# mit-acl/dpgo

Measured on AMD Instinct MI355X. Metric: rbcd_iterations_per_sec, higher is better.
Workload: dtype f64; 1 GPU; synthetic 3-D grid 50x50x40 (100000 poses, 293500 edges), init = perturbed truth; agents=1, agents_per_gpu=1, r=5, d=3, schedule=single agent, poses_per_agent=100000, nnzb_per_agent=687000

## Files before the change

dpgo_amd/csrc/host.h:

```cpp
#pragma once
#include "kernels.h"
#include "handoff.h"
#include "options.h"
#include "taskpool.h"
#include "aggregation.h"

#include <algorithm>
#include <atomic>
#include <chrono>
#include <condition_variable>
#include <functional>
#include <memory>
#include <pthread.h>
#include <sched.h>
#include <mutex>
#include <thread>
#include <type_traits>
#include <cmath>
#include <cstdio>
#include <cstdlib>
#include <cstring>
#include <string>
#include <utility>
#include <vector>
// ... 312 lines not shown
  }
  bool beyond_cache() const {
    return sizeof(double) * ((size_t)Q.nnzb * b * b + 8 * (size_t)n * T) + sizeof(int32_t) * (size_t)Q.nnzb + loop_extra_bytes >
           ((size_t)256 << 20);
  }
  bool persist = false;
  int persist_share = 1;
  int persist_wgs = 0, persist_split = 0, persist_mt = 0;
  int persist_reserved = 0;
  bool persist_failed_once = false;
  bool stream_nt = false;
  bool persist_add = false;
  bool persist_stream_ordered = false;
  struct Pending {
    bool active = false;
    bool launched = false;
    SolvePlan plan;
    BorrowedIterate x;
    dpgo_ropt_result result{};
  } pending;
  DevBuf<PersistCtrl> pctrl;
  bool pctrl_dirty = true;
  DevBuf<unsigned long long> pgran;
  unsigned gran_cleared_at = 0;
  PinBuf<PersistCtrl> hctrl;
  DevBuf<double> partial_mem;
  Partials pE, pA, pB, pH;
  DevBuf<DevState> state_mem;
  StateSlots<DevState> state;
  PinBuf<DevState> hstate;
  PinBuf<unsigned long long> hflag;
  unsigned gen = 0;
  bool saw_rtr_stop = false;
  struct GncEdges {
    int em = 0;
    DevBuf<int32_t> e_p1, e_p2, c_ptr, c_edge;
    DevBuf<double> e_R, e_t, e_kappa, e_tau, e_w, e_rsq, q_base;
    DevBuf<uint8_t> e_fixed, c_kind, e_role;
    DevBuf<int32_t> e_slot;
    DevBuf<int32_t> g_ptr, g_edge;
    DevBuf<uint8_t> g_kind;
    DevBuf<double> c_base;
    int n_shared_edges = 0;
    DevBuf<RobustPartial> r_partial;
    DevBuf<RobustStatsDev> r_stats;
    EdgeDev dev() const {
      return EdgeDev{e_p1, e_p2, e_R, e_t, e_kappa, e_tau, e_fixed, e_role, e_slot, e_w, e_rsq, em};
    }
  } gnc;
  size_t vec_bytes() const { return (size_t)n * T * sizeof(double); }
  int grid() const { return std::min(pose_tiles(n, b), cap_u); }
  int cap_u = kMaxGrid, cap_h = kMaxGrid;
  int cap_u_ml = kMaxGrid;
  int grid_u(bool ml_mode) const { return std::min(pose_tiles(n, b), ml_mode ? cap_u_ml : cap_u); }
  int split = 1;
  int grid_s() const { return std::min(pose_tiles(n, b, split), tcg_sym ? cap_hs : cap_h); }
  int cap_restrict = kMaxGrid, cap_post = kMaxGrid;
  int grid_restrict() const { return std::min(pose_tiles(n, b, split), cap_restrict); }
  int grid_post() const { return std::min(pose_tiles(n, b, split), cap_post); }
  int cap_outer_sym = kMaxGrid;
  int grid_outer_sym() const { return std::min(pose_tiles(n, b), cap_outer_sym); }
  int cap_spmm_sym = kMaxGrid;
  int grid_spmm_sym() const { return std::min(pose_tiles(n, b), cap_spmm_sym); }
  int grid_spmm() const { return std::min(pose_tiles(n, b, split), kMaxGrid); }
  int grid_flat() const {
    size_t total = (size_t)n * T;
// ... 112 lines not shown
```

dpgo_amd/csrc/kernels/common.h:

```cpp
#pragma once


constexpr int kBlock = 256;
constexpr int kWaves = kBlock / 64;
constexpr int kMaxGrid = 1024;
constexpr int kPartialCap = 1024;
constexpr int kNP = 4;

enum : int { TCG_NEGCURV = 0, TCG_EXCREGION = 1, TCG_LCON = 2, TCG_SCON = 3, TCG_MAXITER = 4 };

struct DevState {
  double f1, ngf, Delta, Delta_max, tol;
  double f2, rho, fInit, gnInit;
  double xqx, xg;
  int outer_iter, rtr_stop, accepted_last, n_accept;
  int accept_tiny, pad0;
  double z_r, d_Pd, e_Pd, e_Pe, norm_r0, alpha, theta, kappa;
  double d_Hd;
  int tcg_j, tcg_done, tcg_status, max_inner;
  int n_hess, min_inner;
};

__device__ __forceinline__ void publish_progress(unsigned long long* hflag, unsigned gen, const DevState& st) {
  if (hflag) {
    const unsigned long long w = ((unsigned long long)gen << 32) |
                                 ((unsigned long long)((unsigned)st.tcg_j & 0xFFFFFFu) << 8) |
                                 (st.rtr_stop ? 2ull : 0ull) | (st.tcg_done ? 1ull : 0ull);
    __hip_atomic_store(hflag, w, __ATOMIC_RELAXED, __HIP_MEMORY_SCOPE_SYSTEM);
  }
}

__device__ __forceinline__ unsigned state_gen(DevState& st, unsigned gen) {
  if (gen) st.pad0 = (int)gen;
  return (unsigned)st.pad0;
}

#define DPGO_STATE_FIELDS(X)                                                                              \
  X(f1) X(ngf) X(Delta) X(Delta_max) X(tol) X(f2) X(rho) X(fInit) X(gnInit) X(xqx) X(xg) X(outer_iter)      \
  X(rtr_stop) X(accepted_last) X(n_accept) X(accept_tiny) X(pad0) X(z_r) X(d_Pd) X(e_Pd) X(e_Pe) X(norm_r0) \
  X(alpha) X(theta) X(kappa) X(d_Hd) X(tcg_j) X(tcg_done) X(tcg_status) X(max_inner) X(n_hess) X(min_inner)
__device__ __forceinline__ void load_state(DevState& st, const DevState* __restrict__ p) {
#define X(f) st.f = p->f;
  DPGO_STATE_FIELDS(X)
#undef X
}
__device__ __forceinline__ void store_state(DevState* __restrict__ p, const DevState& st) {
#define X(f) p->f = st.f;
  DPGO_STATE_FIELDS(X)
#undef X
}

template <int D, int R, int SPLIT = 1>
struct Geo {
  static constexpr int B = D + 1;
  static constexpr int T = B * R;
  static constexpr int BB = B * B;
  static constexpr int LPP = B * SPLIT;
  static constexpr int G = 64 / LPP;
  static constexpr int P = G * kWaves;
};
// ... 692 lines not shown
```

dpgo_amd/csrc/kernels/multilevel.h:

```cpp
#pragma once


struct AggMap {
  const int32_t* lab;
  int k;
  __device__ __forceinline__ int of(int i) const { return lab ? lab[i] : i / k; }
};

template <int D, int R>
__global__ __launch_bounds__(kBlock) void k_ml_presmooth(const double* __restrict__ V, const double* __restrict__ dinv,
                                                         double omega, double* __restrict__ OUT,
                                                         const DevState* __restrict__ gate, int n) {
  using GEO = Geo<D, R>;
  if (gate && (gate->tcg_done || gate->rtr_stop)) return;
  __shared__ double sm[kWaves][GEO::G][GEO::T];
  const LaneId L = lane_id<D>();
  const int ntiles = (n + GEO::P - 1) / GEO::P;
  const TileIter ti_ = tile_iter(ntiles);
  for (int tile = ti_.first; tile < ti_.last; tile += ti_.step) {
    const int i = tile * GEO::P + L.wave * GEO::G + L.g;
    const bool ok = (L.g < GEO::G) && (i < n);
    const size_t off = (size_t)i * GEO::T + L.c * R;
    double* vs = ok ? &sm[L.wave][L.g][0] : nullptr;
    double v[R], z[R];
// ... 21 lines not shown
};
template <int D, int R, int SPLIT>
struct RestrictWaves {
  static constexpr int kMin = (SPLIT == 1 && D == 3 && R <= 5) ? DPGO_RESTRICT_WAVES : 1;
};
template <int D, int R, int SPLIT, class MAT = BsrDev, class PT = double, class XT = double>
__global__ __launch_bounds__(kBlock) __attribute__((amdgpu_waves_per_eu(RestrictWaves<D, R, SPLIT>::kMin, 8))) void k_ml_restrict(MAT A, const XT* __restrict__ x1,
                                                        const double* __restrict__ r, const PT* __restrict__ Pb,
                                                        double shift, int k, double* __restrict__ rc,
                                                        float* __restrict__ rc32,
                                                        const double* __restrict__ dinv_next, double omega,
                                                        double* __restrict__ x1c, const DevState* gate,
                                                        int n, XT* __restrict__ res_out = nullptr,
                                                        double* __restrict__ tbuf = nullptr,
                                                        const int32_t* __restrict__ tpos = nullptr,
                                                        TcgStopCheck stop = TcgStopCheck()) {
  using GEO = Geo<D, R, SPLIT>;
  DPGO_TL_TILES_DECL;
  if (gate && (gate->tcg_done || gate->rtr_stop)) return;
  DPGO_STAMP_ENTRY_IN(g_tl_restrict);
  __shared__ double res_s[kWaves][GEO::G][GEO::T];
  __shared__ double t_s[GEO::P][GEO::T];
  const LaneId L = lane_id<D, SPLIT>();
  const int ntiles = (n + GEO::P - 1) / GEO::P;
  const TileIter ti_ = tile_iter(ntiles);
  if (stop.state && blockIdx.x == gridDim.x - 1) {
    double rr_sum[1];
    load_partials<1>(stop.pin, stop.nb, rr_sum, &t_s[0][0]);
    if (threadIdx.x == 0) {
      const DevState* st = stop.state;
      const double norm_r = sqrt(rr_sum[0]), nr0 = st->norm_r0, theta = st->theta, kappa = st->kappa;
      const double pw = (theta == 1.0) ? nr0 : pow(nr0, theta);
      const int j = st->tcg_j;
      if (j >= st->min_inner && norm_r <= nr0 * (pw < kappa ? pw : kappa)) {
        stop.state->tcg_status = (kappa < pw) ? TCG_LCON : TCG_SCON;
        stop.state->tcg_done = 1;
        if (stop.hflag) {
          const unsigned g_ = stop.gen ? stop.gen : (unsigned)st->pad0;
          const unsigned long long w = ((unsigned long long)g_ << 32) |
                                       ((unsigned long long)((unsigned)j & 0xFFFFFFu) << 8) | 1ull;
          __hip_atomic_store(stop.hflag, w, __ATOMIC_RELAXED, __HIP_MEMORY_SCOPE_SYSTEM);
        }
      }
    }
    __syncthreads();
  }
  DPGO_STAMP_AT_IN(g_tl_restrict, 1);
  for (int tk = ti_.first; tk < ti_.last; tk += ti_.step) {
    DPGO_STAMP_TILE_IN(g_tl_restrict, 0);
    const int tile = tile_of(A, tk);
    const int lp = L.wave * GEO::G + L.g;
    const int i = tile * GEO::P + lp;
    const bool okp = (L.g < GEO::G) && (i < n);
    const bool ok = okp && (L.s == 0);
    const size_t off = (size_t)i * GEO::T + L.c * R;
    double h[R];
    q_gather<D, R, SPLIT>(A, x1, i, L.s, L.c, okp, h);
    DPGO_TL_USE(h[0]);
    DPGO_STAMP_TILE_IN(g_tl_restrict, 1);
    if (ok) {
      XT xr[R];
      double rr[R];
#pragma unroll
      for (int a = 0; a < R; ++a) xr[a] = x1[off + a];
      load_col<R>(r + off, rr);
#pragma unroll
      for (int a = 0; a < R; ++a) h[a] = rr[a] - h[a] - shift * (double)xr[a];
      store_col<R>(&res_s[L.wave][L.g][L.c * R], h);
      if (res_out) store_col_t<R>(res_out + off, h);
    }
    wave_sync();
    DPGO_STAMP_TILE_IN(g_tl_restrict, 2);
    if (L.s == 0 && L.g < GEO::G) {
      double t[R];
#pragma unroll
// ... 793 lines not shown
```

dpgo_amd/csrc/solve.hip:

```cpp
#include "host.h"

namespace dpgo_host {

int launch_tcg_update(dpgo_problem_s* p, const double* dinv, int first, double* z_out,
                      double ml_omega) {
  const bool ml_mode = ml_omega > 0.0;
  const int g = p->grid_u(ml_mode);
  if (!first) CHK(sums_ready(p->pA));
  double* pb = nullptr;
  CHK(sums_out(p->pB, g, &pb));
  double* zt = z_out ? z_out : p->z;
  float* z32 = (ml_omega > 0.0 && !p->ml.empty() && z_out == p->ml[0].x1 && p->ml_vec32_active()) ? p->ml[0].x1f : nullptr;
  CHK(dispatch_dr(p->d, p->r, [&](auto Dc, auto Rc) {
    constexpr int D = decltype(Dc)::value, R = decltype(Rc)::value;
    const bool def = p->dirs_on;
    auto go = [&](auto kernel, auto... z32_arg) {
      return launch(kernel, g, 0, p->stream, p->x1, p->g1, dinv, def ? nullptr : p->delta.get(), p->Hd,
                    def ? nullptr : p->eta.get(), p->rr, zt, p->pA.in(), p->pA.count(), pb, p->state.in(),
                    p->state.out(), first, p->n, p->hflag, p->gen, ml_omega, def ? p->dirs_coef.get() : nullptr,
                    z32_arg...);
    };
    if constexpr (Span<D, R, 1>::kOk) {
      if (def) return go(ml_mode ? k_tcg_update_span<D, R, 1, 1> : k_tcg_update_span<D, R, 0, 1>, z32);
      return go(ml_mode ? k_tcg_update_span<D, R, 1> : k_tcg_update_span<D, R, 0>, z32);
// ... 257 lines not shown
  HIPC(hipGetLastError());
  *used = true;
  return DPGO_OK;
}

void persist_report(dpgo_problem_s* p) {
  if (!options().persist_verbose) return;
  const double it = std::max<double>(1.0, (double)p->hctrl->ticks[4]);
  std::fprintf(stderr,
               "dpgo_hip: persistent tCG: %u workgroups (%d lane groups per pose, %d tiles each)%s, %u iterations; per "
               "iteration (us): Hessian phase %.2f, all-reduce %.2f, update phase %.2f, all-reduce %.2f; per solve (us): "
               "set-up + initial statistics %.1f, first updates %.1f, retraction / trial point / rho test %.1f\n",
               p->hctrl->members, p->persist_split, p->persist_mt, p->hctrl->error ? " TIMED OUT" : "", p->hctrl->iters,
               0.01 * (double)p->hctrl->ticks[0] / it, 0.01 * (double)p->hctrl->ticks[1] / it,
               0.01 * (double)p->hctrl->ticks[2] / it, 0.01 * (double)p->hctrl->ticks[3] / it,
               0.01 * (double)p->hctrl->ticks[5], 0.01 * (double)p->hctrl->ticks[6], 0.01 * (double)p->hctrl->ticks[7]);
}

int rtr_outer_iteration(dpgo_problem_s* p, const dpgo_ropt_params* prm, const double* dinv, Counters& cnt,
                        bool poll_at_end) {
  p->gen += 1;
  const bool add = prm->precond == DPGO_PRECOND_ADDITIVE;
  const bool ml = prm->precond == DPGO_PRECOND_MULTILEVEL || add;
  if (add) cnt.vcycle_for_additive = true;
  auto update = [&](int first) -> int {
    if (ml) {
      CHK(launch_tcg_update(p, dinv, first, p->ml[0].x1, p->ml_omega));
      const bool early_stop = options().ml_early_stop != 0;
      return launch_ml_tail(p, p->x1, p->rr, p->z, &p->pB, p->state.in(), early_stop && !first);
    }
    return launch_tcg_update(p, dinv, first);
  };
  CHK(update(1));
  const int max_inner = prm->RTR_tCG_iterations;
  auto step = [&](int j) -> int {
    CHK(launch_tcg_hess(p, j == 0 ? 1 : 0));
    return update(0);
  };
  if (max_inner <= 0) CHK(launch_tcg_hess(p, 1));
  bool done = false;
  if (prm->tcg_poll_interval > 0) {
    const int poll = prm->tcg_poll_interval;
    int j = 0;
    while (j < max_inner) {
      const int chunk = (max_inner - j) < poll ? (max_inner - j) : poll;
      for (int c = 0; c < chunk; ++c) CHK(step(j + c));
      j += chunk;
      CHK(poll_state(p));
      if (p->hstate->tcg_done || p->hstate->rtr_stop) {
        done = true;
        break;
      }
    }
  } else {
    int kAhead = ml ? 2 : 4;
    if (options().tcg_ahead > 0) kAhead = std::max(2, options().tcg_ahead);
    int enq = 0, last_j = -1;
    auto t_progress = std::chrono::steady_clock::now();
    while (true) {
      const unsigned long long w = __atomic_load_n(p->hflag.get(), __ATOMIC_ACQUIRE);
      int dev_j = 0;
      if ((unsigned)(w >> 32) == p->gen) {
        dev_j = (int)((w >> 8) & 0xFFFFFFu);
        if (w & 3ull) {
          done = true;
          if (w & 2ull) p->saw_rtr_stop = true;
          break;
        }
      }
      if (enq >= max_inner) break;
      if (dev_j != last_j) {
        last_j = dev_j;
        t_progress = std::chrono::steady_clock::now();
      }
      if (enq < dev_j + kAhead) {
        CHK(step(enq));
        enq += 1;
      } else {
        __builtin_ia32_pause();
        if (std::chrono::duration<double>(std::chrono::steady_clock::now() - t_progress).count() > 60.0) {
          HIPC(hipStreamSynchronize(p->stream));
          return fail(DPGO_ERR_HIP, "tCG progress word did not advance for 60 s");
        }
      }
    }
  }
  if (!done) CHK(launch_tcg_hess(p, 0));
  if (p->saw_rtr_stop) return DPGO_OK;
  const bool rho_exact = options().rho_exact != 0;
  CHK(launch_retract(p, p->x1, p->eta, 1.0, p->x2, p->state.in(), rho_exact ? nullptr : p->rr.get(),
                     rho_exact ? nullptr : p->g1.get(), p->dirs_on));
  CHK(launch_grad(p, p->x2, p->g2, p->S2, nullptr, p->state.in(), p->tcg_sym && outer_sym_enabled()));
  cnt.spmm += 1;
  if (rho_exact) {
    CHK(launch_hess(p, p->x1, p->S1, p->eta, p->g1, p->Hd, p->state.in(), 0, p->tcg_sym && outer_sym_enabled()));
    cnt.spmm += 1;
  }
  CHK(launch_rtr_update(p));
  if (poll_at_end) CHK(poll_state(p));
  return DPGO_OK;
}

constexpr int kAutoUnitsJacobi = 10, kAutoUnitsAdditive = 13, kAutoSetupUnits = 2800, kAutoMinProducts = 6;
constexpr int kAutoUnitsAdditive2 = 22;
int auto_units_jacobi(dpgo_problem_s* p) {
  const int share = std::max(1, p->persist_share);
  if (share == 1 || !p->persist) return kAutoUnitsJacobi;
  const int cap = persist_capacity(p->device), limit = cap - cap / 5;
// ... 111 lines not shown
                     (prm->precond == DPGO_PRECOND_ADDITIVE || prm->precond == DPGO_PRECOND_BLOCK_JACOBI ||
                      prm->precond == DPGO_PRECOND_NONE);
  return DPGO_OK;
}

int one_launch_enqueue(dpgo_problem_s* p, const SolvePlan& plan, bool* used) {
  return launch_rtr_persistent(p, &plan.prm, plan.dinv, used, plan.prm.precond == DPGO_PRECOND_ADDITIVE);
}

int one_launch_collect(dpgo_problem_s* p, const SolvePlan& plan, dpgo_ropt_result* res, bool* ok) {
  *ok = false;
  std::memset(res, 0, sizeof(*res));
  res->tCGStatus = DPGO_TCG_MAXITER;
  HIPC(hipStreamSynchronize(p->stream));
  persist_report(p);
  if (p->hstate->rtr_stop == kPersistPoison || p->hctrl->error) {
    p->persist_failed_once = true;
    p->pctrl_dirty = true;
    persist_release(p);
    if (options().persist_verbose)
      std::fprintf(stderr, "dpgo_hip: persistent solve timed out; this handle continues with the multi-launch scheme\n");
    return DPGO_OK;
  }
  const DevState& h = *p->hstate;
  res->fInit = h.fInit;
  res->gradNormInit = h.gnInit;
  res->fOpt = h.f1;
  res->gradNormOpt = h.ngf;
  res->tCGStatus = h.outer_iter > 0 ? h.tcg_status : DPGO_TCG_MAXITER;
  res->rtr_iterations = h.outer_iter;
  res->rtr_accepted = h.n_accept;
  res->latest_step_accepted = h.accepted_last;
  res->tcg_iterations = h.n_hess;
  res->precond_used = plan.prm.precond;
  res->spmm_count = 1 + 2 * h.outer_iter + h.n_hess;
  if (plan.is_auto) auto_update(p, &plan.prm, plan.prm.precond, h.n_hess);
  res->success = 1;
  res->elapsedMs = 1e3 * std::chrono::duration<double>(std::chrono::steady_clock::now() - plan.t0).count();
  *ok = true;
  return DPGO_OK;
}

int multi_launch_solve(dpgo_problem_s* p, const SolvePlan& plan, dpgo_ropt_result* res) {
  const dpgo_ropt_params* prm = &plan.prm;
  const double* dinv = plan.dinv;
  Counters cnt;
  std::memset(res, 0, sizeof(*res));
  res->tCGStatus = DPGO_TCG_MAXITER;
  p->dirs_on = false;
  if (prm->method == DPGO_METHOD_RTR) CHK(tcg_dirs_ensure(p, prm->RTR_tCG_iterations));
  CHK(launch_grad(p, p->x1, p->g1, p->S1, nullptr, nullptr, prm->method == DPGO_METHOD_RTR && p->tcg_sym && outer_sym_enabled()));
  cnt.spmm += 1;
  CHK(launch_rtr_begin(p, prm->gradnorm_tol, prm->RTR_initial_radius, 5.0 * prm->RTR_initial_radius,
                       prm->RTR_tCG_iterations, prm->accept_tiny_decrease));
  const bool deferred = prm->method == DPGO_METHOD_RTR && prm->RTR_iterations != 1 && prm->tcg_poll_interval <= 0;
  if (!deferred) {
    CHK(poll_state(p));
    res->fInit = p->hstate->fInit;
    res->gradNormInit = p->hstate->gnInit;
  } else {
    p->hstate->rtr_stop = 0;
  }
  int n_hess_total = 0;
  int shrink_tries = 0;

  if (prm->method == DPGO_METHOD_RTR) {
    if (!p->hstate->rtr_stop) {
      if (prm->RTR_iterations == 1) {
        double radius = prm->RTR_initial_radius;
        int total_steps = 0;
        while (true) {
          shrink_tries += 1;
          p->hstate->Delta = radius;
          p->hstate->Delta_max = radius;
          p->hstate->outer_iter = 0;
          CHK(push_state(p));
          p->saw_rtr_stop = false;
          CHK(rtr_outer_iteration(p, prm, dinv, cnt, true));
          if (p->hstate->accepted_last) break;
          if (total_steps > 10) break;
          radius /= 4.0;
// ... 14 lines not shown
          res->gradNormInit = p->hstate->gnInit;
        }
      }
      res->tCGStatus = p->hstate->tcg_status;
      res->rtr_iterations = (prm->RTR_iterations == 1) ? shrink_tries : p->hstate->outer_iter;
      res->rtr_accepted = p->hstate->n_accept;
      res->latest_step_accepted = p->hstate->accepted_last;
      n_hess_total = p->hstate->n_hess;
    }
    res->fOpt = p->hstate->f1;
    res->gradNormOpt = p->hstate->ngf;
  } else if (prm->method == DPGO_METHOD_RGD) {
    const double* step = p->g1;
    if (prm->RGD_use_preconditioner) {
      if (prm->precond == DPGO_PRECOND_MULTILEVEL)
        CHK(launch_ml_apply(p, p->x1, p->g1, p->z));
      else
        CHK(launch_precond(p, p->x1, p->g1, dinv, p->z));
      step = p->z;
    }
    CHK(launch_retract(p, p->x1, step, -prm->RGD_stepsize, p->x2, nullptr));
    HIPC(hipMemcpyAsync(p->x1, p->x2, p->vec_bytes(), hipMemcpyDeviceToDevice, p->stream));
    CHK(launch_grad(p, p->x1, p->g1, p->S1, nullptr));
    cnt.spmm += 1;
    CHK(launch_rtr_begin(p, prm->gradnorm_tol, prm->RTR_initial_radius, 5.0 * prm->RTR_initial_radius,
                         prm->RTR_tCG_iterations, prm->accept_tiny_decrease));
    CHK(poll_state(p));
    res->fOpt = p->hstate->f1;
    res->gradNormOpt = p->hstate->ngf;
  } else {
    return fail(DPGO_ERR_INVALID, "unknown method");
  }
  res->tcg_iterations = n_hess_total;
  res->precond_used = (prm->precond == DPGO_PRECOND_ADDITIVE && cnt.vcycle_for_additive) ? DPGO_PRECOND_MULTILEVEL : prm->precond;
  if (plan.is_auto && prm->method == DPGO_METHOD_RTR) auto_update(p, prm, res->precond_used, n_hess_total);
  res->spmm_count = cnt.spmm + n_hess_total;
  res->success = 1;
  res->elapsedMs = 1e3 * std::chrono::duration<double>(std::chrono::steady_clock::now() - plan.t0).count();
  return DPGO_OK;
}

int run_optimize(dpgo_problem_s* p, const dpgo_ropt_params* prm, dpgo_ropt_result* res) {
  struct SlotGuard {
    dpgo_problem_s* p;
    ~SlotGuard() { persist_release(p); }
  } slot_guard{p};
  SolvePlan plan;
  bool used = false, ok = false;
  CHK(plan_solve(p, prm, &plan));
  if (plan.one_launch) CHK(one_launch_enqueue(p, plan, &used));
  if (used) CHK(one_launch_collect(p, plan, res, &ok));
  return ok ? DPGO_OK : multi_launch_solve(p, plan, res);
}

int BorrowedIterate::begin(dpgo_problem_s* p, double* X_dev) {
  if (!aligned8(X_dev)) return fail(DPGO_ERR_INVALID, "iterate not 8-byte aligned");
  own_x1 = p->x1;
  staged = aligned16(X_dev) ? nullptr : X_dev;
  if (staged) HIPC(hipMemcpyAsync(own_x1, staged, p->vec_bytes(), hipMemcpyDeviceToDevice, p->stream));
  else p->x1 = X_dev;
  return DPGO_OK;
}
int BorrowedIterate::end(dpgo_problem_s* p, int rc) {
  p->x1 = own_x1;
  if (rc == DPGO_OK && staged) HIPC(hipMemcpyAsync(staged, own_x1, p->vec_bytes(), hipMemcpyDeviceToDevice, p->stream));
  return rc;
// ... 336 lines not shown
  HIPC(hipMemcpyFromSymbol(out, HIP_SYMBOL(g_timeline), sizeof(long long) * 32));
  return DPGO_OK;
}
int dpgo_debug_timeline_tiles(long long* out ) {
  HIPC(hipDeviceSynchronize());
  HIPC(hipMemcpyFromSymbol(out, HIP_SYMBOL(g_tl_tiles), sizeof(long long) * 3 * 64));
  return DPGO_OK;
}
#endif


int dpgo_problem_persistent_info(dpgo_problem_t p, int* enabled, int* workgroups, int* last_members, int* last_iterations,
                                 int* last_layout) {
  if (!p) return fail(DPGO_ERR_INVALID, "null handle");
  if (enabled) *enabled = (p->persist && !p->persist_failed_once) ? 1 : 0;
  if (workgroups) *workgroups = p->persist_wgs;
  if (last_members) *last_members = p->hctrl ? (int)p->hctrl->members : 0;
  if (last_iterations) *last_iterations = p->hctrl ? (int)p->hctrl->iters : 0;
  if (last_layout) *last_layout = (p->hctrl && p->hctrl->members) ? p->persist_split * 16 + p->persist_mt : 0;
  return DPGO_OK;
}


int dpgo_problem_persistent_phases(dpgo_problem_t p, double us_per_iteration[4], int* iterations) {
  if (!p || !us_per_iteration) return fail(DPGO_ERR_INVALID, "null handle / pointer");
  const double it = p->hctrl ? (double)p->hctrl->ticks[4] : 0.0;
  for (int k = 0; k < 4; ++k)
    us_per_iteration[k] = (p->hctrl && it > 0.0 && p->hctrl->members) ? 0.01 * (double)p->hctrl->ticks[k] / it : 0.0;
  if (iterations) *iterations = (p->hctrl && p->hctrl->members) ? (int)p->hctrl->iters : 0;
  return DPGO_OK;
}


int dpgo_problem_set_persistent(dpgo_problem_t p, int enable) {
  if (!p) return fail(DPGO_ERR_INVALID, "null handle");
  if (enable && persist_geometry(p, persist_capacity(p->device)).wgs <= 0)
    return fail(DPGO_ERR_UNSUPPORTED, "block too large for the persistent tCG kernel (at most 2 tiles on each of 256 workgroups)");
  p->persist = enable != 0;
  if (enable) p->persist_failed_once = false;
  return DPGO_OK;
}


int dpgo_problem_tcg_kernel_info(dpgo_problem_t p, int* symmetric, int* split, int* stream_nt) {
  CHK(check_ready(p));
  CHK(resolve_tcg_storage(p));
  if (symmetric) *symmetric = p->tcg_sym ? 1 : 0;
  if (split) *split = p->tcg_sym ? 1 : p->split;
  if (stream_nt) *stream_nt = (p->stream_nt && (p->tcg_sym || p->split == 1)) ? 1 : 0;
  return DPGO_OK;
}


int dpgo_problem_tcg_directions_info(dpgo_problem_t p, int* deferred, int* slots) {
  if (!p) return fail(DPGO_ERR_INVALID, "null handle");
  if (deferred) *deferred = p->dirs_on ? 1 : 0;
  if (slots) *slots = p->dirs ? p->dirs_cap : 0;
  return DPGO_OK;
}

}
```

dpgo_amd/lib.py:

```python
from __future__ import annotations

import ctypes as C
import os
import sys
from typing import Optional

import numpy as np

_HERE = os.path.dirname(os.path.abspath(__file__))
LIB_PATH = os.environ.get("DPGO_LIB") or os.path.join(_HERE, "libdpgo_hip.so")

OK, ERR_INVALID, ERR_HIP, ERR_UNSUPPORTED, ERR_STATE = 0, 1, 2, 3, 4
METHOD_RTR, METHOD_RGD = 0, 1
PRECOND_NONE, PRECOND_BLOCK_JACOBI, PRECOND_MULTILEVEL, PRECOND_AUTO, PRECOND_ADDITIVE = 0, 1, 2, 3, 4
PRECOND_NAMES = ["none", "jacobi", "multilevel", "auto", "additive"]
ML_P_BLOCKS, ML_A_ROWPTR, ML_A_COLIDX, ML_A_VALUES, ML_DENSE_INVERSE, ML_AGG_LABELS, ML_AP_NNZB = 0, 1, 2, 3, 4, 5, 6
ML_RESTRICT_PARTIALS = 7
TCG_STATUS = ["NEGCURVTURE", "EXCREGION", "LCON", "SCON", "MAXITER"]


class DpgoError(RuntimeError):
    def __init__(self, code: int, msg: str):
        super().__init__("dpgo_hip error %d: %s" % (code, msg))
        self.code = code
# ... 146 lines not shown
    "dpgo_problem_tcg_kernel_info": ([_P, C.POINTER(_I), C.POINTER(_I), C.POINTER(_I)], _I),
    "dpgo_problem_tcg_directions_info": ([_P, C.POINTER(_I), C.POINTER(_I)], _I),
    "dpgo_bench_spmm_rotating": ([_P, _I, _I, _I, C.POINTER(_D), C.POINTER(_D)], _I),
    "dpgo_bench_hess_rotating": ([_P, _I, _I, _I, C.POINTER(_D)], _I),
    "dpgo_bench_hess": ([_P, _I, _I, C.POINTER(_D)], _I),
    "dpgo_bench_solve": ([_P, C.POINTER(RoptParamsC), _P, _I, _I, C.POINTER(_D), C.POINTER(_D), C.POINTER(_I)], _I),
    "dpgo_bench_iteration_kernels": ([_P, _I, _I, _P], _I),
    "dpgo_manifold_project": ([_I, _I, _I, _P, _P, _I], _I),
    "dpgo_manifold_tangent_project": ([_I, _I, _I, _P, _P, _P, _I], _I),
    "dpgo_manifold_retract": ([_I, _I, _I, _P, _P, _D, _P, _I], _I),
    "dpgo_manifold_project_device": ([_I, _I, _I, _P, _P, _P], _I),
    "dpgo_round_trajectory": ([_I, _I, _I, _P, _P, _P, _I], _I),
    "dpgo_round_trajectory_device": ([_I, _I, _I, _P, _P, _P, _P], _I),
    "dpgo_gather_tiles_device": ([_I, _I, _P, _P, _I, _P, _P], _I),
    "dpgo_locality_order": ([_I, _P, _P, _I, _I, _P], _I),
    "dpgo_locality_order_runs": ([_I, _P, _P, _I, _I, _I, _P], _I),
    "dpgo_permute_tiles_device": ([_I, _I, _I, _P, _P, _P, _I, _P], _I),
    "dpgo_exchange_plan_create": ([C.POINTER(_P), _I, _I, _I, _P, _P, _P, _P, _I], _I),
    "dpgo_exchange_plan_run": ([_P, _P], _I),
    "dpgo_exchange_plan_destroy": ([_P], _I),
    "dpgo_flags_write_device": ([_I, _P, _P, _P], _I),
    "dpgo_flags_wait_device": ([_I, _P, _P, _I, _P], _I),
    "dpgo_flags_wait_device_checked": ([_I, _P, _P, C.c_longlong, _P, _P], _I),
    "dpgo_max_translation_distance_device": ([_I, _I, _I, _P, _P, _P, C.POINTER(_D), _P], _I),
    "dpgo_axpby_project_device": ([_I, _I, _I, _D, _P, _D, _P, _D, _P, _I, _P, _P], _I),
    "dpgo_average_params_default": ([_I, C.POINTER(AverageParamsC)], None),
    "dpgo_neighbor_candidates_device": ([_I, _I, _I, _P, _P, _P, _P, _P, _P, _P, _P, _P, _P], _I),
    "dpgo_robust_average_device": ([_I, _I, _P, _P, _P, _P, C.POINTER(AverageParamsC), _P, _P, _P], _I),
    "dpgo_robust_average": ([_I, _I, _P, _P, _P, _P, C.POINTER(AverageParamsC), _P, _P, _I], _I),
    "dpgo_lift_in_frame_device": ([_I, _I, _I, _P, _P, _P, _P, _P, _P], _I),
    "dpgo_problem_set_persistent": ([_P, _I], _I),
    "dpgo_problem_persistent_info": ([_P, C.POINTER(_I), C.POINTER(_I), C.POINTER(_I), C.POINTER(_I), C.POINTER(_I)], _I),
    "dpgo_problem_persistent_phases": ([_P, _P, C.POINTER(_I)], _I),
    "dpgo_chordal_initialization": ([_I, _I, _I, _P, _P, _P, _P, _P, _P, _D, _I, _P, _P, _I], _I),
    "dpgo_odometry_initialization": ([_I, _I, _I, _P, _P, _P, _P, _P], _I),
    "dpgo_device_malloc": ([C.POINTER(_P), C.c_size_t, _I], _I),
    "dpgo_device_free": ([_P], _I),
    "dpgo_device_memcpy": ([_P, _P, C.c_size_t, _I, _P], _I),
    "dpgo_device_synchronize": ([_P], _I),
    "dpgo_comm_unique_id": ([_P], _I),
    "dpgo_comm_create": ([C.POINTER(_P), _I, _I, _P, _I], _I),
    "dpgo_comm_destroy": ([_P], _I),
    "dpgo_comm_info": ([_P, C.POINTER(_I), C.POINTER(_I)], _I),
    "dpgo_comm_exchange": ([_P, _I, _P, _P, _P, _I, _P, _P, _P, _P], _I),
    "dpgo_comm_allreduce": ([_P, _P, _I, _I, _P], _I),
    "dpgo_comm_broadcast": ([_P, _P, _I, _I, _P], _I),
    "dpgo_build_Q_bsr": ([_I, _I, _I, _I, _P, _P, _P, _P, _P, _P, _P, _P, _P, _I, _P, _D, _D,
                          C.POINTER(_I), _P, _P, _P], _I),
    "dpgo_build_G_coupling": ([_I, _I, _I, _I, _P, _P, _P, _P, _P, _P, _P, _P, _P, _P,
                               C.POINTER(_I), _P, _P, _P], _I),
    "dpgo_debug_reduction_primitives": ([_I, _I, _I, _P, _P, _P, _P, _P], _I),
    "dpgo_debug_live_allocations": ([C.POINTER(C.c_longlong), C.POINTER(C.c_longlong)], _I),
    "dpgo_certify_params_default": ([C.POINTER(CertifyParamsC)], None),
    "dpgo_problem_certify": ([_P, _P, C.POINTER(CertifyParamsC), C.POINTER(CertifyResultC), _P], _I),
    "dpgo_problem_certify_device": ([_P, _P, C.POINTER(CertifyParamsC), C.POINTER(CertifyResultC), _P], _I),
    "dpgo_problem_certificate_apply": ([_P, _P, _P, _P], _I),
    "dpgo_certify_escape_device": ([_P, _I, _P, _P, _D, _P, C.POINTER(_D)], _I),
    "dpgo_team_certify_device": ([C.POINTER(TeamMemberC), _I, _P, C.POINTER(CertifyParamsC),
                                  C.POINTER(TeamCertifyResultC), _P], _I),
    "dpgo_team_certificate_apply_device": ([C.POINTER(TeamMemberC), _I, _P, _P, _P], _I),
    "dpgo_team_certificate_apply_gram_device": ([C.POINTER(TeamMemberC), _I, _P, _P, _P, _P], _I),
    "dpgo_team_eval_device": ([C.POINTER(TeamMemberC), _I, _P, C.POINTER(_D), C.POINTER(_D), _P], _I),
    "dpgo_team_escape_device": ([C.POINTER(TeamMemberC), _I, _I, _P, _P, _D, _P, C.POINTER(TeamEscapeResultC)], _I),
}

_lib: Optional[C.CDLL] = None
# ... 60 lines not shown
```

dpgo_amd/solver.py:

```python
from __future__ import annotations

import ctypes as C
from dataclasses import dataclass
from typing import Dict, Optional, Tuple

import numpy as np

from . import lib as L
from .measurements import RelativeSEMeasurements


@dataclass
class ROptParameters:
    method: str = "RTR"
    verbose: bool = False
    gradnorm_tol: float = 1e-2
    RGD_stepsize: float = 1e-3
    RGD_use_preconditioner: bool = True
    RTR_iterations: int = 3
    RTR_tCG_iterations: int = 50
    RTR_initial_radius: float = 100.0
    precond: str = "auto"
    precond_shift: float = 1e-1
    accept_tiny_decrease: bool = True
# ... 410 lines not shown
        L.check(self._lib.dpgo_problem_set_G_coupling(self._h, len(slots), len(colidx), L.ptr(rowptr),
                                                      L.ptr(colidx) if len(colidx) else None,
                                                      L.ptr(vals) if len(colidx) else None, L.ptr(G0)))
        return slots

    def updateLinearMatrixFromNeighbors(self, nbr_tiles_dev) -> None:
        L.check(self._lib.dpgo_problem_update_G_from_neighbors_device(self._h, L.ptr(nbr_tiles_dev)))
        self._g_obj = None

    def setPersistent(self, enable: bool = True) -> None:
        L.check(self._lib.dpgo_problem_set_persistent(self._h, int(enable)))

    def tcgKernelInfo(self) -> dict:
        v = [C.c_int(0) for _ in range(3)]
        L.check(self._lib.dpgo_problem_tcg_kernel_info(self._h, *[C.byref(x) for x in v]))
        w = [C.c_int(0) for _ in range(2)]
        L.check(self._lib.dpgo_problem_tcg_directions_info(self._h, *[C.byref(x) for x in w]))
        return dict(symmetric=bool(v[0].value), split=v[1].value, stream_nt=bool(v[2].value),
                    directions=bool(w[0].value), direction_slots=w[1].value)

    def persistentInfo(self) -> dict:
        v = [C.c_int(0) for _ in range(5)]
        L.check(self._lib.dpgo_problem_persistent_info(self._h, *[C.byref(x) for x in v]))
        out = dict(zip(("enabled", "workgroups", "last_members", "last_iterations"), (x.value for x in v[:4])))
        out["last_split"], out["last_tiles"] = v[4].value // 16, v[4].value % 16
        return out

    def persistentPhases(self) -> dict:
        v = (C.c_double * 4)()
        it = C.c_int(0)
        L.check(self._lib.dpgo_problem_persistent_phases(self._h, v, C.byref(it)))
        return dict(hessian=v[0], reduce_after_hessian=v[1], update=v[2], reduce_after_update=v[3], iterations=it.value)

    def multilevelPath(self) -> dict:
        v = C.c_int(0)
        L.check(self._lib.dpgo_problem_multilevel_path(self._h, C.byref(v)))
        return dict(ap=bool(v.value & 1), packed_dense=bool(v.value & 2))

    def multilevelCoarseBits(self, bits=None) -> int:
        v = C.c_int(-1 if bits is None else int(bits))
        L.check(self._lib.dpgo_problem_multilevel_coarse_bits(self._h, C.byref(v)))
        return int(v.value)

    def multilevelOperatorBits(self, bits=None) -> dict:
        v, act = C.c_int(-1 if bits is None else int(bits)), C.c_int(0)
        L.check(self._lib.dpgo_problem_multilevel_operator_bits(self._h, C.byref(v), C.byref(act)))
        return dict(bits=int(v.value), active=bool(act.value & 1), vectors=bool(act.value & 2), dense=bool(act.value & 4))

    def setupMultilevel(self, ks=None, omega: float = 0.7, shift: float = 1e-1, coarse_bits=None) -> dict:
        self.refresh()
        if coarse_bits is not None:
            self.multilevelCoarseBits(coarse_bits)
        ks = L.i32(ks if ks is not None else [])
        L.check(self._lib.dpgo_problem_setup_multilevel(self._h, len(ks), L.ptr(ks) if len(ks) else None,
                                                        float(omega), float(shift)))
        return self.multilevelInfo()

    def setSpmmVariant(self, variant: str = "auto") -> str:
        self.refresh()
        names = {"auto": 0, "plain": 1, "symmetric": 2}
        if variant not in names:
            raise ValueError("variant must be one of %s" % sorted(names))
        v = C.c_int(0)
        L.check(self._lib.dpgo_problem_set_spmm_variant(self._h, names[variant], C.byref(v)))
        return "symmetric" if v.value == 2 else "plain"

# ... 281 lines not shown
```

include/dpgo_hip.h:

```cpp
#ifndef DPGO_HIP_H
#define DPGO_HIP_H

#include <stddef.h>
#include <stdint.h>

#ifdef __cplusplus
extern "C" {
#endif

#define DPGO_OK 0
#define DPGO_ERR_INVALID 1
#define DPGO_ERR_HIP 2
#define DPGO_ERR_UNSUPPORTED 3
#define DPGO_ERR_STATE 4

#define DPGO_METHOD_RTR 0
#define DPGO_METHOD_RGD 1

#define DPGO_PRECOND_NONE 0
#define DPGO_PRECOND_BLOCK_JACOBI 1
#define DPGO_PRECOND_MULTILEVEL 2
#define DPGO_PRECOND_AUTO 3
#define DPGO_PRECOND_ADDITIVE 4

// ... 149 lines not shown

int dpgo_optimize_device_many(int count, const dpgo_problem_t* handles, const dpgo_ropt_params* params,
                              double* const* X_dev, const double* const* nbr_tiles_dev, void* after_stream,
                              dpgo_ropt_result* results);
int dpgo_problem_eval_terms_device_many(int count, const dpgo_problem_t* handles, const double* const* X_dev,
                                        const double* const* nbr_tiles_dev, void* after_stream, double* terms);

int dpgo_spmm_device(dpgo_problem_t h, const double* V_dev, double* OUT_dev, int add_G);
int dpgo_problem_eval_device(dpgo_problem_t h, const double* X_dev, double* f, double* gradnorm);
int dpgo_problem_eval_terms_device(dpgo_problem_t h, const double* X_dev, double* xqx, double* xg, double* g2);
#define DPGO_SPMM_AUTO 0
#define DPGO_SPMM_PLAIN 1
#define DPGO_SPMM_SYMMETRIC 2
int dpgo_problem_set_spmm_variant(dpgo_problem_t h, int variant, int* in_use);
int dpgo_problem_tcg_kernel_info(dpgo_problem_t h, int* symmetric, int* split, int* stream_nt);
int dpgo_problem_tcg_directions_info(dpgo_problem_t h, int* deferred, int* slots);
int dpgo_bench_spmm(dpgo_problem_t h, int reps, int warmup, double* avg_ms);
int dpgo_bench_spmm_rotating(dpgo_problem_t h, int nsets, int reps, int warmup, double* avg_ms, double* set_bytes);
int dpgo_bench_hess(dpgo_problem_t h, int reps, int warmup, double* avg_ms);
int dpgo_bench_solve(dpgo_problem_t h, const dpgo_ropt_params* params, const double* X0_dev, int reps, int warmup,
                     double* avg_ms, double* avg_products, int* persistent);
int dpgo_bench_hess_rotating(dpgo_problem_t h, int nsets, int reps, int warmup, double* avg_ms);
int dpgo_bench_iteration_kernels(dpgo_problem_t h, int reps, int warmup, double out_ms[5]);

int dpgo_debug_reduction_primitives(int workgroups, int pay, int steps, const double* in_dev, const double* pay_in_dev,
                                    double* sums_dev, double* pay_out_dev, double* rows_out_dev);

int dpgo_debug_live_allocations(long long* buffers, long long* bytes);

int dpgo_problem_set_persistent(dpgo_problem_t h, int enable);
int dpgo_problem_persistent_info(dpgo_problem_t h, int* enabled, int* workgroups, int* last_members,
                                 int* last_iterations, int* last_layout);
int dpgo_problem_persistent_phases(dpgo_problem_t h, double us_per_iteration[4], int* iterations);

int dpgo_locality_order(int n, const int32_t* rowptr, const int32_t* colidx, int nparts, int align, int32_t* new_index);
int dpgo_locality_order_runs(int n, const int32_t* rowptr, const int32_t* colidx, int nparts, int align, int run,
                             int32_t* new_index);
int dpgo_permute_tiles_device(int r, int d, int n, const int32_t* new_index_dev, const double* in_dev, double* out_dev,
                              int forward, void* stream);

int dpgo_chordal_initialization(int d, int n, int m, const int32_t* p1, const int32_t* p2, const double* R,
                                const double* t, const double* kappa, const double* tau, double tol, int max_iter,
                                double* T_host, int iters_out[2], int device);
int dpgo_odometry_initialization(int d, int n, int m, const int32_t* p1, const int32_t* p2, const double* R,
                                 const double* t, double* T_host);

#define DPGO_COPY_H2D 0
#define DPGO_COPY_D2H 1
#define DPGO_COPY_D2D 2
int dpgo_device_malloc(void** out, size_t bytes, int device);
int dpgo_device_free(void* p);
int dpgo_device_memcpy(void* dst, const void* src, size_t bytes, int kind, void* stream);
int dpgo_device_synchronize(void* stream);

#define DPGO_COMM_ID_BYTES 128
#define DPGO_COMM_SUM 0
#define DPGO_COMM_MAX 1
typedef struct dpgo_comm_s* dpgo_comm_t;
int dpgo_comm_unique_id(char id[DPGO_COMM_ID_BYTES]);
int dpgo_comm_create(dpgo_comm_t* out, int nranks, int rank, const char id[DPGO_COMM_ID_BYTES], int device);
int dpgo_comm_destroy(dpgo_comm_t c);
int dpgo_comm_info(dpgo_comm_t c, int* nranks, int* rank);
int dpgo_comm_exchange(dpgo_comm_t c, int nsend, const int* send_peer, const double* const* send_dev,
                       const int* send_count, int nrecv, const int* recv_peer, double* const* recv_dev,
                       const int* recv_count, void* stream);
int dpgo_comm_allreduce(dpgo_comm_t c, double* buf_dev, int count, int op, void* stream);
// ... 153 lines not shown
```

Measured before the change: 273.5 it/s.

## Gate host tCG step enqueueing on device go tickets for multilevel early stop

The restrict kernel now publishes a progress word on every stop check, carrying either a done bit or a new 'go' bit. When multilevel early stop is on with two levels, the host enqueues the next tCG step only after the device signals go for the previous step, instead of running a fixed number of steps ahead. The aim is to stop enqueuing dead iterations that would just exit early after convergence, at the cost of a host-device round trip that can leave the GPU idle between steps. Feed counters and an API to read them are added for diagnostics.

```diff
diff --git a/dpgo_amd/csrc/host.h b/dpgo_amd/csrc/host.h
--- a/dpgo_amd/csrc/host.h
+++ b/dpgo_amd/csrc/host.h
@@ -368,6 +368,9 @@
   PinBuf<unsigned long long> hflag;
   unsigned gen = 0;
   bool saw_rtr_stop = false;
+  struct FeedCounts {
+    long long steps = 0, runs = 0, runs_fed = 0, products = 0;
+  } feed;
   struct GncEdges {
     int em = 0;
     DevBuf<int32_t> e_p1, e_p2, c_ptr, c_edge;
diff --git a/dpgo_amd/csrc/kernels/common.h b/dpgo_amd/csrc/kernels/common.h
--- a/dpgo_amd/csrc/kernels/common.h
+++ b/dpgo_amd/csrc/kernels/common.h
@@ -21,11 +21,14 @@
   int n_hess, min_inner;
 };
 
+constexpr unsigned long long kProgressDone = 1ull, kProgressRtrStop = 2ull, kProgressGo = 4ull;
+__device__ __forceinline__ unsigned long long progress_word(unsigned gen, int tcg_j, unsigned long long bits) {
+  return ((unsigned long long)gen << 32) | ((unsigned long long)((unsigned)tcg_j & 0xFFFFFFu) << 8) | bits;
+}
 __device__ __forceinline__ void publish_progress(unsigned long long* hflag, unsigned gen, const DevState& st) {
   if (hflag) {
-    const unsigned long long w = ((unsigned long long)gen << 32) |
-                                 ((unsigned long long)((unsigned)st.tcg_j & 0xFFFFFFu) << 8) |
-                                 (st.rtr_stop ? 2ull : 0ull) | (st.tcg_done ? 1ull : 0ull);
+    const unsigned long long w =
+        progress_word(gen, st.tcg_j, (st.rtr_stop ? kProgressRtrStop : 0ull) | (st.tcg_done ? kProgressDone : 0ull));
     __hip_atomic_store(hflag, w, __ATOMIC_RELAXED, __HIP_MEMORY_SCOPE_SYSTEM);
   }
 }
diff --git a/dpgo_amd/csrc/kernels/multilevel.h b/dpgo_amd/csrc/kernels/multilevel.h
--- a/dpgo_amd/csrc/kernels/multilevel.h
+++ b/dpgo_amd/csrc/kernels/multilevel.h
@@ -77,15 +77,15 @@
       const double norm_r = sqrt(rr_sum[0]), nr0 = st->norm_r0, theta = st->theta, kappa = st->kappa;
       const double pw = (theta == 1.0) ? nr0 : pow(nr0, theta);
       const int j = st->tcg_j;
-      if (j >= st->min_inner && norm_r <= nr0 * (pw < kappa ? pw : kappa)) {
+      const bool met = j >= st->min_inner && norm_r <= nr0 * (pw < kappa ? pw : kappa);
+      if (met) {
         stop.state->tcg_status = (kappa < pw) ? TCG_LCON : TCG_SCON;
         stop.state->tcg_done = 1;
-        if (stop.hflag) {
-          const unsigned g_ = stop.gen ? stop.gen : (unsigned)st->pad0;
-          const unsigned long long w = ((unsigned long long)g_ << 32) |
-                                       ((unsigned long long)((unsigned)j & 0xFFFFFFu) << 8) | 1ull;
-          __hip_atomic_store(stop.hflag, w, __ATOMIC_RELAXED, __HIP_MEMORY_SCOPE_SYSTEM);
-        }
+      }
+      if (stop.hflag) {
+        const unsigned g_ = stop.gen ? stop.gen : (unsigned)st->pad0;
+        const unsigned long long w = progress_word(g_, j, met ? kProgressDone : kProgressGo);
+        __hip_atomic_store(stop.hflag, w, __ATOMIC_RELAXED, __HIP_MEMORY_SCOPE_SYSTEM);
       }
     }
     __syncthreads();
diff --git a/dpgo_amd/csrc/solve.hip b/dpgo_amd/csrc/solve.hip
--- a/dpgo_amd/csrc/solve.hip
+++ b/dpgo_amd/csrc/solve.hip
@@ -313,8 +313,11 @@
     return launch_tcg_update(p, dinv, first);
   };
   CHK(update(1));
+  p->feed.runs += 1;
   const int max_inner = prm->RTR_tCG_iterations;
   auto step = [&](int j) -> int {
+    if (j == 0) p->feed.runs_fed += 1;
+    p->feed.steps += 1;
     CHK(launch_tcg_hess(p, j == 0 ? 1 : 0));
     return update(0);
   };
@@ -336,25 +339,30 @@
   } else {
     int kAhead = ml ? 2 : 4;
     if (options().tcg_ahead > 0) kAhead = std::max(2, options().tcg_ahead);
-    int enq = 0, last_j = -1;
+    const bool tickets = ml && !poll_at_end && options().ml_early_stop != 0 && p->ml.size() == 2;
+    int enq = 0;
+    unsigned long long last_w = ~0ull;
     auto t_progress = std::chrono::steady_clock::now();
     while (true) {
       const unsigned long long w = __atomic_load_n(p->hflag.get(), __ATOMIC_ACQUIRE);
+      const bool current = (unsigned)(w >> 32) == p->gen;
       int dev_j = 0;
-      if ((unsigned)(w >> 32) == p->gen) {
+      if (current) {
         dev_j = (int)((w >> 8) & 0xFFFFFFu);
-        if (w & 3ull) {
+        if (w & (kProgressDone | kProgressRtrStop)) {
           done = true;
-          if (w & 2ull) p->saw_rtr_stop = true;
+          if (w & kProgressRtrStop) p->saw_rtr_stop = true;
           break;
         }
       }
       if (enq >= max_inner) break;
-      if (dev_j != last_j) {
-        last_j = dev_j;
+      const unsigned long long w_run = current ? w : 0ull;
+      if (w_run != last_w) {
+        last_w = w_run;
         t_progress = std::chrono::steady_clock::now();
       }
-      if (enq < dev_j + kAhead) {
+      const bool feed = tickets ? (current && (enq == 0 || ((w & kProgressGo) && dev_j >= enq - 1))) : (enq < dev_j + kAhead);
+      if (feed) {
         CHK(step(enq));
         enq += 1;
       } else {
@@ -532,6 +540,8 @@
   res->rtr_accepted = h.n_accept;
   res->latest_step_accepted = h.accepted_last;
   res->tcg_iterations = h.n_hess;
+  p->feed = dpgo_problem_s::FeedCounts();
+  p->feed.products = h.n_hess;
   res->precond_used = plan.prm.precond;
   res->spmm_count = 1 + 2 * h.outer_iter + h.n_hess;
   if (plan.is_auto) auto_update(p, &plan.prm, plan.prm.precond, h.n_hess);
@@ -547,6 +557,7 @@
   Counters cnt;
   std::memset(res, 0, sizeof(*res));
   res->tCGStatus = DPGO_TCG_MAXITER;
+  p->feed = dpgo_problem_s::FeedCounts();
   p->dirs_on = false;
   if (prm->method == DPGO_METHOD_RTR) CHK(tcg_dirs_ensure(p, prm->RTR_tCG_iterations));
   CHK(launch_grad(p, p->x1, p->g1, p->S1, nullptr, nullptr, prm->method == DPGO_METHOD_RTR && p->tcg_sym && outer_sym_enabled()));
@@ -627,6 +638,7 @@
     return fail(DPGO_ERR_INVALID, "unknown method");
   }
   res->tcg_iterations = n_hess_total;
+  p->feed.products = n_hess_total;
   res->precond_used = (prm->precond == DPGO_PRECOND_ADDITIVE && cnt.vcycle_for_additive) ? DPGO_PRECOND_MULTILEVEL : prm->precond;
   if (plan.is_auto && prm->method == DPGO_METHOD_RTR) auto_update(p, prm, res->precond_used, n_hess_total);
   res->spmm_count = cnt.spmm + n_hess_total;
@@ -1029,6 +1041,16 @@
 }
 
 
+int dpgo_problem_feed_counters(dpgo_problem_t p, long long counts[4]) {
+  if (!p || !counts) return fail(DPGO_ERR_INVALID, "null handle / pointer");
+  counts[0] = p->feed.steps;
+  counts[1] = p->feed.runs;
+  counts[2] = p->feed.runs_fed;
+  counts[3] = p->feed.products;
+  return DPGO_OK;
+}
+
+
 int dpgo_problem_set_persistent(dpgo_problem_t p, int enable) {
   if (!p) return fail(DPGO_ERR_INVALID, "null handle");
   if (enable && persist_geometry(p, persist_capacity(p->device)).wgs <= 0)
diff --git a/dpgo_amd/lib.py b/dpgo_amd/lib.py
--- a/dpgo_amd/lib.py
+++ b/dpgo_amd/lib.py
@@ -202,6 +202,7 @@
     "dpgo_problem_set_persistent": ([_P, _I], _I),
     "dpgo_problem_persistent_info": ([_P, C.POINTER(_I), C.POINTER(_I), C.POINTER(_I), C.POINTER(_I), C.POINTER(_I)], _I),
     "dpgo_problem_persistent_phases": ([_P, _P, C.POINTER(_I)], _I),
+    "dpgo_problem_feed_counters": ([_P, _P], _I),
     "dpgo_chordal_initialization": ([_I, _I, _I, _P, _P, _P, _P, _P, _P, _D, _I, _P, _P, _I], _I),
     "dpgo_odometry_initialization": ([_I, _I, _I, _P, _P, _P, _P, _P], _I),
     "dpgo_device_malloc": ([C.POINTER(_P), C.c_size_t, _I], _I),
diff --git a/dpgo_amd/solver.py b/dpgo_amd/solver.py
--- a/dpgo_amd/solver.py
+++ b/dpgo_amd/solver.py
@@ -466,6 +466,11 @@
         L.check(self._lib.dpgo_problem_persistent_phases(self._h, v, C.byref(it)))
         return dict(hessian=v[0], reduce_after_hessian=v[1], update=v[2], reduce_after_update=v[3], iterations=it.value)
 
+    def feedCounters(self) -> dict:
+        v = (C.c_longlong * 4)()
+        L.check(self._lib.dpgo_problem_feed_counters(self._h, v))
+        return dict(steps=v[0], runs=v[1], runs_fed=v[2], products=v[3], dead_iterations=v[0] - v[3])
+
     def multilevelPath(self) -> dict:
         v = C.c_int(0)
         L.check(self._lib.dpgo_problem_multilevel_path(self._h, C.byref(v)))
diff --git a/include/dpgo_hip.h b/include/dpgo_hip.h
--- a/include/dpgo_hip.h
+++ b/include/dpgo_hip.h
@@ -205,6 +205,7 @@
 int dpgo_problem_persistent_info(dpgo_problem_t h, int* enabled, int* workgroups, int* last_members,
                                  int* last_iterations, int* last_layout);
 int dpgo_problem_persistent_phases(dpgo_problem_t h, double us_per_iteration[4], int* iterations);
+int dpgo_problem_feed_counters(dpgo_problem_t h, long long counts[4]);
 
 int dpgo_locality_order(int n, const int32_t* rowptr, const int32_t* colidx, int nparts, int align, int32_t* new_index);
 int dpgo_locality_order_runs(int n, const int32_t* rowptr, const int32_t* colidx, int nparts, int align, int run,
```

After: 278.3 it/s (median of 6 runs). 1.02x the previous value.
